# automl/TransformersCanDoBayesianInference

Hardware: AMD Instinct MI355X
Metric: synthetic datasets/sec (GP prior, bptt=2000) (higher is better)
Workload: dtype fp16; 1 GPU; priors.fast_gp, bptt=2000, num_features=18, emsize=512, nhead=4, nhid=1024, nlayers=6, 1000 bars (BASELINE.json configs[1]); per_gpu_batch=64, global_batch=64, aggregate_k_gradients=1, aggregate_streams=0, aggregate_stacked=False, seq_len=2000, parallelism=dp1, micro_batch_streams=2, eval_pos=weighted sampler(2000)

## Files before the change

### transformerscandobayesianinference_amd/csrc/attention.hip

```cpp
#include <algorithm>
#include <type_traits>
#include "pfn_device.h"
#include "pfn_kernels.h"

namespace pfn {

template <typename T, int D> struct AttnCfg {
  static constexpr int RB = D * (int)sizeof(T);
  static constexpr int KVB = (sizeof(T) == 2 && D <= 128) ? 64 : 32;
  static constexpr int NKB = KVB / 32;
  static constexpr int NKK = D / 16;
  static constexpr int NDB = D / 32;
  static constexpr int TILE = KVB * RB;
  static constexpr int RS = PadStride<RB>::ROW, CS = PadStride<RB>::COL;
  static constexpr int RIMG = KVB * RS, CIMG = KVB * CS;
  static constexpr int NW = (sizeof(T) == 2 && D <= 128) ? 8 : 4;
  static constexpr int NT = NW * 64;
  static constexpr int QBLK = NW * 32;
};

template <typename T> PFN_DEV Frag<T> load_frag_global(const T* p) {
  Frag<T> f;
  if constexpr (sizeof(T) == 2) {
    f.v = *reinterpret_cast<const X8<T>*>(p);
// ... 26 lines not shown
    const unsigned w = __builtin_bit_cast(u32x4, f.v)[e >> 1];
    return __builtin_bit_cast(float, (e & 1) ? (w & 0xffff0000u) : (w << 16));
  } else return f.v[e];
}
template <typename T> PFN_DEV float dot8(const Frag<T>& a, const Frag<T>& b) {
  float s = 0.f;
#pragma unroll
  for (int e = 0; e < 8; ++e) s += frag_get(a, e) * frag_get(b, e);
  return s;
}
template <typename T> PFN_DEV f32x4 load4(const T* p) {
  f32x4 r;
  if constexpr (sizeof(T) == 2) {
    X4<T> v = *reinterpret_cast<const X4<T>*>(p);
#pragma unroll
    for (int e = 0; e < 4; ++e) r[e] = (float)v[e];
  } else r = *reinterpret_cast<const f32x4*>(p);
  return r;
}
template <typename T> PFN_DEV void store4(T* p, f32x4 x) {
  if constexpr (sizeof(T) == 2) {
    X4<T> v;
#pragma unroll
    for (int e = 0; e < 4; ++e) v[e] = (T)x[e];
    *reinterpret_cast<X4<T>*>(p) = v;
  } else *reinterpret_cast<f32x4*>(p) = x;
}
PFN_DEV float fast_exp2(float x) { return __builtin_amdgcn_exp2f(x); }

struct AttnBlock { int blk, hd, b; };
PFN_DEV AttnBlock attn_block(int nblk, int H) {
  const int nwg = gridDim.x, bid = blockIdx.x;
  const int q = nwg >> 3, r = nwg & 7, xcd = bid & 7;
  const int id = (xcd < r ? xcd * (q + 1) : r * (q + 1) + (xcd - r) * q) + (bid >> 3);
  AttnBlock o;
  o.blk = id % nblk;
  const int bh = id / nblk;
  o.hd = bh % H;
  o.b = bh / H;
  return o;
}

PFN_DEV AttnBlock attn_block_ragged_last(int nblk, int nfull, int H) {
  if (nfull == nblk) return attn_block(nblk, H);
  const int nwg = gridDim.x, bid = blockIdx.x, npairs = nwg / nblk;
  const int q = nwg >> 3, r = nwg & 7, xcd = bid & 7, j = bid >> 3;
  const int n_x = q + (xcd < r ? 1 : 0);
  const int first = xcd < r ? xcd * (q + 1) : r * (q + 1) + (xcd - r) * q;
  const int r_lo = (int)((long)first * npairs / nwg), r_hi = (int)((long)(first + n_x) * npairs / nwg);
  const int f_x = n_x - (r_hi - r_lo);
  const int f_off = first - r_lo;
  AttnBlock o;
  int pair;
  if (j < f_x) { const int id = f_off + j; pair = id / nfull; o.blk = id % nfull; }
  else { pair = r_lo + (j - f_x); o.blk = nfull; }
  o.hd = pair % H;
  o.b = pair / H;
  return o;
}

typedef __attribute__((address_space(3))) void lvoid_t;
constexpr float LOG2E = 1.4426950408889634f;
constexpr float LN2 = 0.6931471805599453f;
constexpr float RESCALE_THR = 6.f;

PFN_DEV int cache_sep(const int* sep_of, int b, int sep) { return sep_of ? min(max(sep_of[b], 0), sep) : sep; }
PFN_DEV int cache_live_splits(const int* sep_of, int b, int sep, int split_keys, int nsplit) {
  return sep_of ? max(1, min(nsplit, (cache_sep(sep_of, b, sep) + split_keys - 1) / split_keys)) : nsplit;
}

template <typename T> PFN_DEV Frag<T> acc_to_frag_m1(const f32x16& acc, int c, const float (&add8)[8]) {
  static_assert(sizeof(T) == 2, "16-bit operands");
  typedef X2<T> x2;
  const x2 a0 = {(T)(acc[8 * c + 0] + add8[0]), (T)(acc[8 * c + 1] + add8[1])}, a1 = {(T)(acc[8 * c + 2] + add8[2]), (T)(acc[8 * c + 3] + add8[3])};
  const x2 b0 = {(T)(acc[8 * c + 4] + add8[4]), (T)(acc[8 * c + 5] + add8[5])}, b1 = {(T)(acc[8 * c + 6] + add8[6]), (T)(acc[8 * c + 7] + add8[7])};
  const auto r0 = __builtin_amdgcn_permlane32_swap(__builtin_bit_cast(unsigned, a0), __builtin_bit_cast(unsigned, b0), false, false);
  const auto r1 = __builtin_amdgcn_permlane32_swap(__builtin_bit_cast(unsigned, a1), __builtin_bit_cast(unsigned, b1), false, false);
  const u32x4 w = {r0[0], r1[0], r0[1], r1[1]};
  Frag<T> f;
  f.v = __builtin_bit_cast(X8<T>, w);
  return f;
}

template <typename T, int D, bool DROP = false, int DV = D, bool FUSEQ = false, bool CACHE = false>
__global__ __launch_bounds__((AttnCfg<T, D>::NT)) void attn_fwd_kernel(AttnArgs a) {
  static_assert(!CACHE || (!DROP && !FUSEQ), "predict against a cache: no dropout, Q from qkv");
  operand_store_mode<T>();
  using C = AttnCfg<T, D>;
  using CV = AttnCfg<T, DV>;
  static_assert(C::KVB == CV::KVB && D % DV == 0, "V slices share the K tile's key count");
  extern __shared__ __attribute__((aligned(16))) char smem_raw[];
  LdsPtr smem = lds_cast(smem_raw);
  auto Kt = [&](int buf) { return smem + buf * C::RIMG; };
  auto Vt = [&](int buf) { return smem + 2 * C::RIMG + buf * CV::CIMG; };
  constexpr int NVB = 4;
  const int vcol0 = DV == D ? 0 : (int)blockIdx.y * DV;

  AttnBlock wg = attn_block((a.S + C::QBLK - 1) / C::QBLK - a.q_begin / C::QBLK, a.H);
  wg.blk += a.q_begin / C::QBLK;
  const int b = wg.b, hd = wg.hd;
  const int wave = threadIdx.x >> 6, lane = threadIdx.x & 63, h = lane >> 5, li = lane & 31;
  const int lag = (C::NW == 8 && (a.pingpong & 1)) ? (wave >> 2) : 0;
  const long rs = 3L * a.E;
  const T* base = reinterpret_cast<const T*>(a.qkv) + (long)b * a.S * rs;
  const T* Qp = base + hd * D;
  const T* Kp = base + a.E + hd * D;
  const T* Vp = base + 2 * a.E + hd * D + vcol0;
  const int qi = wg.blk * C::QBLK + wave * 32 + li;
  const bool qvalid = qi < a.S;
  const int qc = min(qi, a.S - 1);
  const int k_lo = CACHE ? (int)blockIdx.z * a.split_keys : 0;
  const int sep = CACHE ? min(cache_sep(a.sep_of, b, a.sep) - k_lo, a.split_keys) : a.sep_of ? a.sep_of[b] : a.sep;
  if constexpr (CACHE) { if (blockIdx.z > 0 && sep <= 0) return; }
  const long kld = CACHE ? a.kv_ld : rs;
  const T* Ksrc = CACHE ? reinterpret_cast<const T*>(a.kv) + b * a.kv_sb + k_lo * kld + hd * D : Kp;
  const T* Vsrc = CACHE ? Ksrc + a.E + vcol0 : Vp;
  if (a.q_from_sep && (wg.blk + 1) * C::QBLK <= sep / 256 * 256) return;
  const float scale_log2 = rsqrtf((float)D) * LOG2E;
  const unsigned dseed = DROP ? dropout_pair_seed(a.drop_seed, b * a.H + hd) : 0u;
  const unsigned dthr = DROP ? dropout_threshold(a.p_drop) : 0u;

  Frag<T> qf[C::NKK];
  if constexpr (FUSEQ) {
    static_assert(sizeof(T) == 2 && D <= 128 && C::NW == 8, "fused Q projection: the 8-wave 16-bit configurations");
    constexpr int EC = 128, WS = EC * 2 + 16, WIMG = D * WS;
    static_assert(2 * WIMG <= 2 * C::RIMG + 4 * CV::CIMG, "W_q chunk buffers must fit the (idle) K / V tile buffers");
    const T* xrow = reinterpret_cast<const T*>(a.xq) + ((long)b * a.S + qc) * a.E;
    const T* wq_h = reinterpret_cast<const T*>(a.wq) + (long)(hd * D) * a.E;
    f32x16 qa[C::NDB];
#pragma unroll
    for (int db = 0; db < C::NDB; ++db)
#pragma unroll
      for (int r = 0; r < 16; ++r) qa[db][r] = 0.f;
    TileStage<T, D, EC * 2, C::NT> sw;
    const int nch = a.E / EC;
    sw.issue(wq_h, a.E, D, EC);
    sw.template commit_p<WS>(smem);
    __syncthreads();
    for (int ch = 0; ch < nch; ++ch) {
      const lds_char* wimg = smem + (ch & 1) * WIMG;
      if (ch + 1 < nch) sw.issue(wq_h + (ch + 1) * EC, a.E, D, EC);
      Frag<T> xf[EC / 16];
#pragma unroll
      for (int ks = 0; ks < EC / 16; ++ks) xf[ks] = load_frag_global<T>(xrow + ch * EC + ks * 16 + 8 * h);
#pragma unroll
      for (int ks = 0; ks < EC / 16; ++ks) {
        Frag<T> wf[C::NDB];
#pragma unroll
        for (int db = 0; db < C::NDB; ++db) wf[db] = load_frag_row_p<T, WS>(wimg, db * 32 + li, ks * 16);
#pragma unroll
        for (int db = 0; db < C::NDB; ++db) qa[db] = mma32(wf[db], xf[ks], qa[db]);
      }
      if (ch + 1 < nch) sw.template commit_p<WS>(smem + ((ch + 1) & 1) * WIMG);
      __syncthreads();
    }
    const float* bq = a.bq + hd * D;
    T* qout = reinterpret_cast<T*>(const_cast<void*>(a.qkv)) + (long)b * a.S * rs + hd * D + (long)qc * rs;
#pragma unroll
    for (int db = 0; db < C::NDB; ++db)
#pragma unroll
      for (int c = 0; c < 2; ++c) {
        const f32x4 b0 = *reinterpret_cast<const f32x4*>(bq + db * 32 + 16 * c + 4 * h), b1 = *reinterpret_cast<const f32x4*>(bq + db * 32 + 16 * c + 8 + 4 * h);
        const float add8[8] = {b0[0], b0[1], b0[2], b0[3], b1[0], b1[1], b1[2], b1[3]};
        qf[2 * db + c] = acc_to_frag_m1<T>(qa[db], c, add8);
        if (a.q_store && qvalid) *reinterpret_cast<X8<T>*>(qout + (2 * db + c) * 16 + 8 * h) = qf[2 * db + c].v;
      }
  } else {
#pragma unroll
    for (int kk = 0; kk < C::NKK; ++kk) qf[kk] = load_frag_global<T>(Qp + (long)qc * rs + kk * 16 + 8 * h);
  }

  const bool is_test = CACHE || qc >= sep;
  const bool wave_has_test = CACHE ? blockIdx.z == 0 : wg.blk * C::QBLK + wave * 32 + 31 >= sep;
  float m = -1e30f, lsum = 0.f;
  f32x16 o[CV::NDB];
#pragma unroll
  for (int db = 0; db < CV::NDB; ++db)
#pragma unroll
    for (int r = 0; r < 16; ++r) o[db][r] = 0.f;
  if (wave_has_test) {
    float part = 0.f;
#pragma unroll
    for (int kk = 0; kk < C::NKK; ++kk) part += dot8(qf[kk], load_frag_global<T>(Kp + (long)qc * rs + kk * 16 + 8 * h));
    part += __shfl_xor(part, 32, 64);
    m = is_test ? part * scale_log2 : -1e30f;
    lsum = (is_test && h == 0) ? 1.f : 0.f;
#pragma unroll
    for (int db = 0; db < CV::NDB; ++db)
#pragma unroll
      for (int rg = 0; rg < 4; ++rg) {
        f32x4 v = load4<T>(Vp + (long)qc * rs + db * 32 + 8 * rg + 4 * h);
#pragma unroll
        for (int e = 0; e < 4; ++e) o[db][4 * rg + e] = (is_test && (!DROP || dropout_keep(dseed, (unsigned)qc, (unsigned)qc, dthr))) ? v[e] : 0.f;
      }
  }

  const int nfull = sep / C::KVB;
  const int ntiles = (sep + C::KVB - 1) / C::KVB;
  TileStage<T, C::KVB, C::RB, C::NT> sk;
  TileStage<T, C::KVB, CV::RB, C::NT> sv;
  if (ntiles > 0) {
    sk.issue(Ksrc, kld, sep, D);
    sv.issue(Vsrc, kld, sep, DV);
    sk.template commit_p<C::RS>(Kt(0));
    sv.template commit_p<CV::CS>(Vt(0));
    if (ntiles > 1) {
      sk.issue(Ksrc + (long)C::KVB * kld, kld, sep - C::KVB, D);
      sv.issue(Vsrc + (long)C::KVB * kld, kld, sep - C::KVB, DV);
    }
  }
  __syncthreads();

  constexpr int NPF = C::KVB / 16;
  Frag<T> pf[NPF];
  auto pv_prev = [&](int vb) __attribute__((always_inline)) {
    const lds_char* vt = Vt(vb);
#pragma unroll
    for (int c = 0; c < NPF; ++c)
#pragma unroll
      for (int db = 0; db < CV::NDB; ++db)
        o[db] = mma32(load_frag_tr_p<T, CV::CS, 2>(vt, c * 16, db * 32), pf[c], o[db]);
  };
  int vb_prev = 0, vb_cur = 0;
  for (int t = 0; t < ntiles; ++t) {
    const int k0 = t * C::KVB;
    const lds_char* kt = Kt(t & 1);
    Frag<T> kfr[C::NKK][C::NKB];
#pragma unroll
    for (int kk = 0; kk < C::NKK; ++kk)
#pragma unroll
      for (int kb = 0; kb < C::NKB; ++kb) kfr[kk][kb] = load_frag_row_p<T, C::RS>(kt, kb * 32 + li, kk * 16);
    PFN_PIN_LDS_MFMA();
    f32x16 st[C::NKB];
#pragma unroll
    for (int kb = 0; kb < C::NKB; ++kb)
#pragma unroll
      for (int r = 0; r < 16; ++r) st[kb][r] = 0.f;
#pragma unroll
    for (int kk = 0; kk < C::NKK; ++kk)
#pragma unroll
      for (int kb = 0; kb < C::NKB; ++kb) st[kb] = mma32(kfr[kk][kb], qf[kk], st[kb]);
    PFN_PIN_LDS_MFMA();
    const int vb_next = vb_cur == NVB - 1 ? 0 : vb_cur + 1;
    sk.template commit_p<C::RS>(Kt((t + 1) & 1));
    sv.template commit_p<CV::CS>(Vt(vb_next));
    if (t + 2 < ntiles) {
      const long k2 = k0 + 2 * C::KVB;
      sk.issue(Ksrc + k2 * kld, kld, sep - (int)k2, D);
      sv.issue(Vsrc + k2 * kld, kld, sep - (int)k2, DV);
    }
    if (t == nfull) {
#pragma unroll
      for (int kb = 0; kb < C::NKB; ++kb)
#pragma unroll
        for (int r = 0; r < 16; ++r)
          if (k0 + kb * 32 + acc_row(r, lane) >= sep) st[kb][r] = -INFINITY;
    }
    float mx = -INFINITY;
#pragma unroll
    for (int kb = 0; kb < C::NKB; ++kb)
#pragma unroll
      for (int r = 0; r < 16; ++r) mx = fmaxf(mx, st[kb][r]);
    mx = fmaxf(mx, __shfl_xor(mx, 32, 64));
    const float mc = mx * scale_log2;
    if (__builtin_amdgcn_ballot_w64(mc > m + RESCALE_THR) != 0) {
      const float m_new = fmaxf(m, mc);
      const float alpha = fast_exp2(m - m_new);
      m = m_new;
      lsum *= alpha;
#pragma unroll
      for (int db = 0; db < CV::NDB; ++db)
#pragma unroll
        for (int r = 0; r < 16; ++r) o[db][r] *= alpha;
      if (t > 0) {
#pragma unroll
        for (int c = 0; c < NPF; ++c)
#pragma unroll
          for (int e = 0; e < 8; ++e) pf[c].set(e, frag_get(pf[c], e) * alpha);
      }
    }
    if (lag) __syncthreads();
    if (t > 0) {
      float rsum = 0.f;
#pragma unroll
      for (int kb = 0; kb < C::NKB; ++kb)
#pragma unroll
        for (int r = 0; r < 16; ++r) {
          const float p = fast_exp2(__builtin_fmaf(st[kb][r], scale_log2, -m));
          st[kb][r] = p;
          rsum += p;
        }
      lsum += rsum;
      pv_prev(vb_prev);
    } else {
      float rsum = 0.f;
#pragma unroll
      for (int kb = 0; kb < C::NKB; ++kb)
#pragma unroll
        for (int r = 0; r < 16; ++r) {
          const float p = fast_exp2(__builtin_fmaf(st[kb][r], scale_log2, -m));
          st[kb][r] = p;
          rsum += p;
        }
      lsum += rsum;
    }
    if constexpr (DROP) {
#pragma unroll
      for (int kb = 0; kb < C::NKB; ++kb)
#pragma unroll
        for (int r = 0; r < 16; ++r)
          if (!dropout_keep(dseed, (unsigned)qc, (unsigned)(k0 + kb * 32 + acc_row(r, lane)), dthr)) st[kb][r] = 0.f;
    }
#pragma unroll
    for (int c = 0; c < NPF; ++c) pf[c] = acc_to_frag<T>(st[c >> 1], c & 1);
    vb_prev = vb_cur;
    vb_cur = vb_next;
    if (!lag) __syncthreads();
  }
  if (ntiles > 0) pv_prev(vb_prev);

  lsum += __shfl_xor(lsum, 32, 64);
  if constexpr (CACHE) {
    if (gridDim.z > 1) {
      const long prow = ((long)blockIdx.z * a.B + b) * a.S + qc;
      float* out = a.part_o + prow * a.E + hd * D + vcol0;
#pragma unroll
      for (int db = 0; db < CV::NDB; ++db) {
        float v[16];
#pragma unroll
        for (int r = 0; r < 16; ++r) v[r] = o[db][r];
        store_row_block<float>(out + db * 32, v, h, qvalid);
      }
      if (qvalid && h == 0 && vcol0 == 0) *reinterpret_cast<float2*>(a.part_ml + 2 * (prow * a.H + hd)) = make_float2(m, lsum);
      return;
    }
  }
  const float inv = DROP ? 1.f / (lsum * (1.f - a.p_drop)) : 1.f / lsum;
  {
    T* out = reinterpret_cast<T*>(a.ctx) + ((long)b * a.S + qc) * a.E + hd * D + vcol0;
#pragma unroll
    for (int db = 0; db < CV::NDB; ++db) {
      float v[16];
#pragma unroll
      for (int r = 0; r < 16; ++r) v[r] = o[db][r] * inv;
      store_row_block<T>(out + db * 32, v, h, qvalid);
    }
    if ((!CACHE || a.lse) && qvalid && h == 0 && vcol0 == 0) a.lse[((long)b * a.H + hd) * a.S + qi] = (m + __builtin_amdgcn_logf(lsum)) * LN2;
  }
}

template <typename T>
__global__ __launch_bounds__(256) void attn_merge_kernel(AttnArgs a, int nsplit, int D) {
  const long rows = (long)a.B * a.S, c4n = a.E / 4, total = rows * c4n;
  for (long i = (long)blockIdx.x * 256 + threadIdx.x; i < total; i += (long)gridDim.x * 256) {
    const long row = i / c4n;
    const int c = (int)(i - row * c4n) * 4, hd = c / D;
    const int nz = cache_live_splits(a.sep_of, (int)(row / a.S), a.sep, a.split_keys, nsplit);
    float mx = -INFINITY;
    for (int z = 0; z < nz; ++z) mx = fmaxf(mx, a.part_ml[2 * ((z * rows + row) * a.H + hd)]);
    f32x4 acc = {0.f, 0.f, 0.f, 0.f};
    float l = 0.f;
    for (int z = 0; z < nz; ++z) {
      const float2 ml = *reinterpret_cast<const float2*>(a.part_ml + 2 * ((z * rows + row) * a.H + hd));
      const float w = fast_exp2(ml.x - mx);
      l += w * ml.y;
      const f32x4 v = *reinterpret_cast<const f32x4*>(a.part_o + (z * rows + row) * a.E + c);
#pragma unroll
      for (int e = 0; e < 4; ++e) acc[e] += w * v[e];
    }
    const float inv = 1.f / l;
#pragma unroll
    for (int e = 0; e < 4; ++e) acc[e] *= inv;
    store4<T>(reinterpret_cast<T*>(a.ctx) + row * a.E + c, acc);
    if (a.lse && c % D == 0) a.lse[((row / a.S) * a.H + hd) * a.S + row % a.S] = (mx + __builtin_amdgcn_logf(l)) * LN2;
  }
}

template <typename T, int D> struct BwdCacheCfg {
  static constexpr int DQ = (sizeof(T) == 4 && D == 256) ? 128 : D;
  static constexpr int KVB = 32;
  static constexpr int NKK = D / 16, NDQ = DQ / 32, NPF = KVB / 16;
  static constexpr int RB = D * (int)sizeof(T), QB = DQ * (int)sizeof(T);
  static constexpr int RS = PadStride<RB>::ROW, CSQ = PadStride<QB>::COL;
  static constexpr int KROW = KVB * RS, KCOL = KVB * CSQ;
  static constexpr size_t LDS = 2 * KROW + KCOL;
  static constexpr bool PREFETCH = !(sizeof(T) == 4 && D == 256);
};

template <typename T, int D>
__global__ __launch_bounds__((AttnCfg<T, D>::NT)) void attn_bwd_cache_kernel(AttnCacheBwdArgs a) {
  operand_store_mode<T>();
  using C = AttnCfg<T, D>;
  using G = BwdCacheCfg<T, D>;
  extern __shared__ __attribute__((aligned(16))) char smem_raw[];
  LdsPtr smem = lds_cast(smem_raw);
  LdsPtr Krow = smem, Vrow = smem + G::KROW, Kcol = smem + 2 * G::KROW;
  const AttnBlock wg = attn_block((a.S + C::QBLK - 1) / C::QBLK, a.H);
  const int b = wg.b, hd = wg.hd;
  const int wave = threadIdx.x >> 6, lane = threadIdx.x & 63, h = lane >> 5, li = lane & 31;
  const int qcol0 = G::DQ == D ? 0 : (int)blockIdx.y * G::DQ;
  const long rs = 3L * a.E;
  const int qi = wg.blk * C::QBLK + wave * 32 + li;
// ... 870 lines not shown
  const int sep = a.sep_of ? a.sep_of[b] : a.sep;
  const int qbeg = a.q_from_sep ? sep / 256 * 256 : a.q_begin;
  if ((qb + 1) * P::TB <= qbeg) return;
  const float scale = rsqrtf((float)D), scale_log2 = scale * LOG2E;
  const bool drop = a.p_drop > 0.f;
  const unsigned dseed = dropout_pair_seed(a.drop_seed, b * a.H + hd), dthr = dropout_threshold(a.p_drop);
  const float dscale = drop ? 1.f / (1.f - a.p_drop) : 1.f;
  plain_load_tile<D>(Qs, Qp, rs, q0, qbeg, a.S);
  plain_load_tile<D>(Os, dOp, a.E, q0, qbeg, a.S);
  if (t < P::TB) { const int q = min(q0 + t, a.S - 1); Ls[t] = lse_g[q] * LOG2E; Dl[t] = delta_g[q]; }
  f32x4 dq[D / 32];
#pragma unroll
  for (int m = 0; m < D / 32; ++m) dq[m] = f32x4{0.f, 0.f, 0.f, 0.f};
  const int q = q0 + r1;
  const bool qlive = q >= qbeg && q < a.S;
  for (int key0 = 0; key0 < sep; key0 += P::TB) {
    __syncthreads();
    plain_load_tile<D>(Ks, Kp, rs, key0, 0, sep);
    plain_load_tile<D>(Vs, Vp, rs, key0, 0, sep);
    __syncthreads();
    {
      float s[4], dp[4];
      plain_dots<D>(Qs + r1 * P::RS, Os + r1 * P::RS, Ks, Vs, c1, s, dp);
#pragma unroll
      for (int j = 0; j < 4; ++j) {
        const bool live = qlive && key0 + c1 + j < sep;
        const float p = live ? fast_exp2(s[j] * scale_log2 - Ls[r1]) : 0.f;
        const float mf = !drop ? 1.f : dropout_keep(dseed, (unsigned)q, (unsigned)(key0 + c1 + j), dthr) ? dscale : 0.f;
        Ds[r1 * P::PS + c1 + j] = p * (mf * dp[j] - Dl[r1]);
      }
    }
    __syncthreads();
    for (int kj = 0; kj < P::TB; ++kj) {
      const float ds = Ds[r1 * P::PS + kj];
#pragma unroll
      for (int m = 0; m < D / 32; ++m) {
        const f32x4 k4 = *reinterpret_cast<const f32x4*>(Ks + kj * P::RS + c1 + 32 * m);
#pragma unroll
        for (int e = 0; e < 4; ++e) dq[m][e] += ds * k4[e];
      }
    }
  }
  __syncthreads();
  const bool test = qlive && q >= sep;
  const int qc = min(max(q, 0), a.S - 1);
  float tq = 0.f, dpv = 0.f;
  f32x4 kself[D / 32], vself[D / 32];
#pragma unroll
  for (int m = 0; m < D / 32; ++m) {
    kself[m] = *reinterpret_cast<const f32x4*>(Kp + (long)qc * rs + c1 + 32 * m);
    vself[m] = *reinterpret_cast<const f32x4*>(Vp + (long)qc * rs + c1 + 32 * m);
    const f32x4 q4 = *reinterpret_cast<const f32x4*>(Qs + r1 * P::RS + c1 + 32 * m), o4 = *reinterpret_cast<const f32x4*>(Os + r1 * P::RS + c1 + 32 * m);
#pragma unroll
    for (int e = 0; e < 4; ++e) { tq += q4[e] * kself[m][e]; dpv += o4[e] * vself[m][e]; }
  }
#pragma unroll
  for (int off = 1; off < 8; off <<= 1) { tq += __shfl_xor(tq, off, 64); dpv += __shfl_xor(dpv, off, 64); }
  const float p_self = test ? fast_exp2(tq * scale_log2 - Ls[r1]) : 0.f;
  const float mself = !drop ? 1.f : dropout_keep(dseed, (unsigned)max(q, 0), (unsigned)max(q, 0), dthr) ? dscale : 0.f;
  const float ds_self = p_self * (mself * dpv - Dl[r1]);
  if (qlive) {
#pragma unroll
    for (int m = 0; m < D / 32; ++m) {
      const f32x4 q4 = *reinterpret_cast<const f32x4*>(Qs + r1 * P::RS + c1 + 32 * m), o4 = *reinterpret_cast<const f32x4*>(Os + r1 * P::RS + c1 + 32 * m);
      f32x4 xq, xk, xv;
#pragma unroll
      for (int e = 0; e < 4; ++e) { xq[e] = (dq[m][e] + ds_self * kself[m][e]) * scale; xk[e] = ds_self * scale * q4[e]; xv[e] = p_self * mself * o4[e]; }
      *reinterpret_cast<f32x4*>(dbase + (long)q * rs + hd * D + c1 + 32 * m) = xq;
      if (test) {
        *reinterpret_cast<f32x4*>(dbase + (long)q * rs + a.E + hd * D + c1 + 32 * m) = xk;
        *reinterpret_cast<f32x4*>(dbase + (long)q * rs + 2 * a.E + hd * D + c1 + 32 * m) = xv;
      }
    }
  }
}

bool attn_fwd_can_fuse_q(int E, int H, int precision) {
  const int D = H > 0 ? E / H : 0;
  return prec_is16(precision) && (D == 32 || D == 64 || D == 128) && E % 128 == 0;
}
template <typename T, int D, bool DROP> static int launch_fwd_k(const AttnArgs& a, hipStream_t s) {
  using C = AttnCfg<T, D>;
  constexpr int DV = (sizeof(T) == 4 && D == 256) ? 128 : D;
  constexpr size_t lds = 2 * C::RIMG + 4 * AttnCfg<T, DV>::CIMG;
  static_assert(lds <= 160 * 1024, "attention forward: tile buffers exceed the CU's LDS");
  if ((a.S + C::QBLK - 1) / C::QBLK <= a.q_begin / C::QBLK) return PFN_OK;
  const dim3 grid(((a.S + C::QBLK - 1) / C::QBLK - a.q_begin / C::QBLK) * a.H * a.B, D / DV);
  if constexpr (sizeof(T) == 2 && D <= 128 && !DROP) {
    if (a.xq) {
      if (!a.wq || !a.bq || a.E % 128) return PFN_ERR_ARGUMENT;
      static LdsAllowance allowance_q;
      allowance_q.ensure(attn_fwd_kernel<T, D, false, DV, true>, lds);
      ProfScope ps(PFN_PROF_ATTN_FWD + (a.q_begin > 0 ? 1 : 0), s);
      hipLaunchKernelGGL((attn_fwd_kernel<T, D, false, DV, true>), grid, dim3(C::NT), lds, s, a);
      return hipGetLastError() == hipSuccess ? PFN_OK : PFN_ERR_LAUNCH;
    }
  }
  if (a.xq) return PFN_ERR_UNSUPPORTED;
  static LdsAllowance allowance;
  allowance.ensure(attn_fwd_kernel<T, D, DROP, DV>, lds);
  ProfScope ps(PFN_PROF_ATTN_FWD + (a.q_begin > 0 ? 1 : 0), s);
  hipLaunchKernelGGL((attn_fwd_kernel<T, D, DROP, DV>), grid, dim3(C::NT), lds, s, a);
  return hipGetLastError() == hipSuccess ? PFN_OK : PFN_ERR_LAUNCH;
}
template <typename T, int D> static int launch_fwd_t(const AttnArgs& a, hipStream_t s) {
  return a.p_drop > 0.f ? launch_fwd_k<T, D, true>(a, s) : launch_fwd_k<T, D, false>(a, s);
}
static int g_attn_cache_split_cap = 0;
void set_attn_cache_split_cap(int splits) { g_attn_cache_split_cap = std::max(splits, 0); }
template <typename T, int D> static int launch_fwd_cache_t(const AttnArgs& a_in, hipStream_t s) {
  using C = AttnCfg<T, D>;
  constexpr int DV = (sizeof(T) == 4 && D == 256) ? 128 : D;
  constexpr size_t lds = 2 * C::RIMG + 4 * AttnCfg<T, DV>::CIMG;
  AttnArgs a = a_in;
  int nsplit = attn_cache_splits(a.B, a.S, a.E, a.H, a.sep, sizeof(T) == 4 ? PFN_PREC_F32 : PFN_PREC_BF16);
  if (g_attn_cache_split_cap > 0) nsplit = std::min(nsplit, g_attn_cache_split_cap);
  const int ntiles = (a.sep + C::KVB - 1) / C::KVB;
  a.split_keys = nsplit > 1 ? (ntiles + nsplit - 1) / nsplit * C::KVB : std::max(a.sep, 1);
  const int nz = nsplit > 1 ? (a.sep + a.split_keys - 1) / a.split_keys : 1;
  if (nz > 1 && (!a.part_o || !a.part_ml)) return PFN_ERR_ARGUMENT;
  static LdsAllowance allowance;
  allowance.ensure(attn_fwd_kernel<T, D, false, DV, false, true>, lds);
  const dim3 grid(((a.S + C::QBLK - 1) / C::QBLK) * a.H * a.B, D / DV, nz);
  hipLaunchKernelGGL((attn_fwd_kernel<T, D, false, DV, false, true>), grid, dim3(C::NT), lds, s, a);
  if (nz > 1) {
    const long work = (long)a.B * a.S * (a.E / 4);
    hipLaunchKernelGGL(attn_merge_kernel<T>, dim3((unsigned)std::min<long>((work + 255) / 256, 4096)), dim3(256), 0, s, a, nz, D);
  }
  return hipGetLastError() == hipSuccess ? PFN_OK : PFN_ERR_LAUNCH;
}
template <typename T, int D, bool DROP> static int launch_bwd_k(const AttnArgs& a, hipStream_t s) {
  using C = AttnCfg<T, D>;
  const int parts = a.parts ? a.parts : ~0;
  if (parts & ATTN_BWD_DELTA) {
    const long pairs = (long)a.B * a.S * a.H;
    int grid = (int)std::min<long>((pairs + 15) / 16, 4096);
    ProfScope ps(PFN_PROF_ATTN_BWD_DELTA + (a.q_begin > 0 ? 1 : 0), s);
    hipLaunchKernelGGL(attn_delta_kernel<T>, dim3(grid), dim3(256), 0, s, a, D);
  }
  constexpr size_t lds_kv = BwdKvCfg<T, D>::LDS, lds_dq = BwdDqCfg<T, D>::LDS;
  static_assert(lds_kv <= 160 * 1024 && lds_dq <= 160 * 1024, "attention backward: tile buffers exceed the CU's LDS");
  static LdsAllowance allow_kv, allow_dq;
  if ((parts & ATTN_BWD_KV) && a.sep > 0) {
    ProfScope ps(PFN_PROF_ATTN_BWD_KV + (a.q_begin > 0 ? 1 : 0), s);
    allow_kv.ensure(attn_bwd_kv_kernel<T, D, DROP>, lds_kv);
    hipLaunchKernelGGL((attn_bwd_kv_kernel<T, D, DROP>), dim3(((a.sep + C::QBLK - 1) / C::QBLK) * a.H * a.B), dim3(C::NT), lds_kv, s, a);
  }
  if (parts & ATTN_BWD_DQ) {
    if (a.q_from_sep) {
      const int rc = launch_zero_row_prefix_ragged(a.dqkv, a.S, a.B, a.sep_of, 3L * a.E * (long)sizeof(T), (long)a.E * (long)sizeof(T), s);
      if (rc != PFN_OK) return rc;
    } else if (a.q_begin > 0) {
      const int rc = launch_zero_row_prefix(a.dqkv, a.S, a.B, a.q_begin, 3L * a.E * (long)sizeof(T), (long)a.E * (long)sizeof(T), s);
      if (rc != PFN_OK) return rc;
    }
    if ((a.S + C::QBLK - 1) / C::QBLK <= a.q_begin / C::QBLK) return hipGetLastError() == hipSuccess ? PFN_OK : PFN_ERR_LAUNCH;
    allow_dq.ensure(attn_bwd_dq_kernel<T, D, DROP>, lds_dq);
    ProfScope ps(PFN_PROF_ATTN_BWD_DQ + (a.q_begin > 0 ? 1 : 0), s);
    hipLaunchKernelGGL((attn_bwd_dq_kernel<T, D, DROP>), dim3(((a.S + C::QBLK - 1) / C::QBLK - a.q_begin / C::QBLK) * a.H * a.B), dim3(C::NT), lds_dq, s, a);
  }
  return hipGetLastError() == hipSuccess ? PFN_OK : PFN_ERR_LAUNCH;
}
template <typename T, int D> static int launch_bwd_t(const AttnArgs& a, hipStream_t s) {
  return a.p_drop > 0.f ? launch_bwd_k<T, D, true>(a, s) : launch_bwd_k<T, D, false>(a, s);
}
template <int D> static int launch_bwd_plain_f32(const AttnArgs& a, hipStream_t s) {
  using P = BwdPlainCfg<D>;
  static_assert(P::LDS <= 160 * 1024, "plain attention backward: tiles exceed the CU's LDS");
  const int parts = a.parts ? a.parts : ~0;
  if (parts & ATTN_BWD_DELTA) {
    const long pairs = (long)a.B * a.S * a.H;
    int grid = (int)std::min<long>((pairs + 15) / 16, 4096);
    hipLaunchKernelGGL(attn_delta_kernel<float>, dim3(grid), dim3(256), 0, s, a, D);
  }
  static LdsAllowance allow_kv, allow_dq;
  if ((parts & ATTN_BWD_KV) && a.sep > 0) {
    allow_kv.ensure(attn_bwd_plain_kv_kernel<D>, P::LDS);
    hipLaunchKernelGGL(attn_bwd_plain_kv_kernel<D>, dim3(((a.sep + P::TB - 1) / P::TB) * a.H * a.B), dim3(256), P::LDS, s, a);
  }
  if (parts & ATTN_BWD_DQ) {
    if (a.q_from_sep) {
      const int rc = launch_zero_row_prefix_ragged(a.dqkv, a.S, a.B, a.sep_of, 3L * a.E * 4L, (long)a.E * 4L, s);
      if (rc != PFN_OK) return rc;
    } else if (a.q_begin > 0) {
      const int rc = launch_zero_row_prefix(a.dqkv, a.S, a.B, a.q_begin, 3L * a.E * 4L, (long)a.E * 4L, s);
      if (rc != PFN_OK) return rc;
    }
    const int nqb = (a.S + P::TB - 1) / P::TB - a.q_begin / P::TB;
    if (nqb > 0) {
      allow_dq.ensure(attn_bwd_plain_dq_kernel<D>, P::LDS);
      hipLaunchKernelGGL(attn_bwd_plain_dq_kernel<D>, dim3(nqb * a.H * a.B), dim3(256), P::LDS, s, a);
    }
  }
  return hipGetLastError() == hipSuccess ? PFN_OK : PFN_ERR_LAUNCH;
}

// ... 122 lines not shown
```

### transformerscandobayesianinference_amd/csrc/pfn_device.h

```cpp
#pragma once
#include <hip/hip_runtime.h>
#include <stdint.h>

namespace pfn {

typedef __bf16 bf16;
typedef __attribute__((ext_vector_type(8))) __bf16 bf16x8;
typedef __attribute__((ext_vector_type(4))) __bf16 bf16x4;
typedef __attribute__((ext_vector_type(2))) __bf16 bf16x2;
typedef _Float16 f16;
typedef __attribute__((ext_vector_type(8))) _Float16 f16x8;
typedef __attribute__((ext_vector_type(4))) _Float16 f16x4;
typedef __attribute__((ext_vector_type(2))) _Float16 f16x2;
typedef __attribute__((ext_vector_type(16))) float f32x16;
typedef __attribute__((ext_vector_type(4))) float f32x4;
typedef __attribute__((ext_vector_type(2))) float f32x2;
typedef __attribute__((ext_vector_type(4))) unsigned int u32x4;
typedef __attribute__((ext_vector_type(2))) unsigned int u32x2;
template <typename T> struct OpVec;
template <> struct OpVec<bf16> { typedef bf16x8 x8; typedef bf16x4 x4; typedef bf16x2 x2; };
template <> struct OpVec<f16> { typedef f16x8 x8; typedef f16x4 x4; typedef f16x2 x2; };
template <> struct OpVec<float> { typedef f32x4 x8; typedef f32x4 x4; typedef f32x2 x2; };
template <typename T> using X8 = typename OpVec<T>::x8;
template <typename T> using X4 = typename OpVec<T>::x4;
// ... 183 lines not shown
      if (valid) *reinterpret_cast<f32x4*>(row_block + 8 * rg + 4 * h) = f32x4{v[4 * rg], v[4 * rg + 1], v[4 * rg + 2], v[4 * rg + 3]};
  }
}

template <typename T> PFN_DEV void store_frag_pair_blocked(T* block, const Frag<T>& f0, const Frag<T>& f1, int j, int h, bool valid) {
  char* base = reinterpret_cast<char*>(block);
  if constexpr (sizeof(T) == 2) {
#pragma unroll
    for (int p = 0; p < 2; ++p) {
      const u32x4 d = __builtin_bit_cast(u32x4, p == 0 ? f0.v : f1.v);
      const auto r0 = __builtin_amdgcn_permlane32_swap(d[0], d[2], false, false);
      const auto r1 = __builtin_amdgcn_permlane32_swap(d[1], d[3], false, false);
      const u32x4 w = {r0[0], r1[0], r0[1], r1[1]};
      if (valid) __builtin_nontemporal_store(w, reinterpret_cast<u32x4*>(base + ((p * 32 + j) * 2 + h) * 16));
    }
  } else {
#pragma unroll
    for (int p = 0; p < 2; ++p) {
      const Frag<T>& f = p == 0 ? f0 : f1;
#pragma unroll
      for (int sub = 0; sub < 2; ++sub)
        if (valid) __builtin_nontemporal_store(f32x4{f.v[4 * sub], f.v[4 * sub + 1], f.v[4 * sub + 2], f.v[4 * sub + 3]},
                                               reinterpret_cast<f32x4*>(base + (((2 * p + sub) * 32 + j) * 2 + h) * 16));
    }
  }
}
template <typename T> PFN_DEV int blocked_chunk_row(int w) { return (w >> 1) & 31; }
template <typename T> PFN_DEV int blocked_chunk_col(int w) {
  if constexpr (sizeof(T) == 2) return 16 * (w >> 6) + 8 * (w & 1);
  else return 8 * (w >> 6) + 4 * (w & 1);
}

typedef __amdgpu_buffer_rsrc_t BufRsrc;
PFN_DEV BufRsrc make_rsrc(const void* base, long bytes) {
  const int n = bytes > 0x7ffffff0L ? 0x7ffffff0 : (bytes < 0 ? 0 : (int)bytes);
  return __builtin_amdgcn_make_buffer_rsrc(const_cast<void*>(base), 0, n, 0x00020000);
}
PFN_DEV u32x4 buf_load16(BufRsrc r, int byte_offset) { return __builtin_amdgcn_raw_buffer_load_b128(r, byte_offset, 0, 0); }
constexpr int BUF_OOB = 0x7ffffff0;

struct DmaRsrc { u32x4 w; };
PFN_DEV DmaRsrc make_dma_rsrc(const void* base, long bytes) {
  const unsigned long long p = (unsigned long long)base;
  const int n = bytes > 0x7ffffff0L ? 0x7ffffff0 : (bytes < 0 ? 0 : (int)bytes);
  DmaRsrc r;
  r.w[0] = __builtin_amdgcn_readfirstlane((unsigned)p);
  r.w[1] = __builtin_amdgcn_readfirstlane((unsigned)(p >> 32) & 0xffffu);
  r.w[2] = __builtin_amdgcn_readfirstlane((unsigned)n);
  r.w[3] = 0x00020000u;
  return r;
}
PFN_DEV void dma_rsrc_advance(DmaRsrc& r, unsigned bytes) {
  const unsigned long long b = (((unsigned long long)r.w[1] << 32) | r.w[0]) + bytes;
  r.w[0] = (unsigned)b;
  r.w[1] = (unsigned)(b >> 32);
  r.w[2] = (unsigned)max((int)r.w[2] - (int)bytes, 0);
}
PFN_DEV void dma16(const DmaRsrc& r, LdsPtr lds_dst_uniform, int byte_offset) {
  unsigned keep;
  const unsigned dst = __builtin_amdgcn_readfirstlane((unsigned)(unsigned long long)lds_dst_uniform);
  const u32x4 w = {(unsigned)__builtin_amdgcn_readfirstlane(r.w[0]), (unsigned)__builtin_amdgcn_readfirstlane(r.w[1]),
                   (unsigned)__builtin_amdgcn_readfirstlane(r.w[2]), (unsigned)__builtin_amdgcn_readfirstlane(r.w[3])};
  asm volatile("s_mov_b32 %0, m0\n\ts_mov_b32 m0, %1\n\ts_nop 0\n\tbuffer_load_dwordx4 %2, %3, 0 offen lds\n\ts_mov_b32 m0, %0"
               : "=&s"(keep) : "s"(dst), "v"(byte_offset), "s"(w) : "memory");
}
PFN_DEV void dma4(const DmaRsrc& r, LdsPtr lds_dst_uniform, int byte_offset) {
  unsigned keep;
  const unsigned dst = __builtin_amdgcn_readfirstlane((unsigned)(unsigned long long)lds_dst_uniform);
  const u32x4 w = {(unsigned)__builtin_amdgcn_readfirstlane(r.w[0]), (unsigned)__builtin_amdgcn_readfirstlane(r.w[1]),
                   (unsigned)__builtin_amdgcn_readfirstlane(r.w[2]), (unsigned)__builtin_amdgcn_readfirstlane(r.w[3])};
  asm volatile("s_mov_b32 %0, m0\n\ts_mov_b32 m0, %1\n\ts_nop 0\n\tbuffer_load_dword %2, %3, 0 offen lds\n\ts_mov_b32 m0, %0"
               : "=&s"(keep) : "s"(dst), "v"(byte_offset), "s"(w) : "memory");
}
PFN_DEV void dma16_global(const void* src, LdsPtr lds_dst_uniform) {
  unsigned keep;
  const unsigned dst = __builtin_amdgcn_readfirstlane((unsigned)(unsigned long long)lds_dst_uniform);
  asm volatile("s_mov_b32 %0, m0\n\ts_mov_b32 m0, %1\n\ts_nop 0\n\tglobal_load_lds_dwordx4 %2, off\n\ts_mov_b32 m0, %0"
               : "=&s"(keep) : "s"(dst), "v"(src) : "memory");
}
template <int N> PFN_DEV void wait_vm_barrier() {
  __builtin_amdgcn_s_waitcnt(0x0070 | (N & 15) | ((N >> 4) << 14));
  asm volatile("s_waitcnt vmcnt(%0) lgkmcnt(0)\n\ts_barrier" :: "n"(N) : "memory");
}
PFN_DEV void dma_wait_all() {
  __builtin_amdgcn_s_waitcnt(0x0F70);
  asm volatile("s_waitcnt vmcnt(0)" ::: "memory");
}

template <typename T, int ROWS, int RB, int NT> struct TileStageBuf {
  static constexpr int NCH = RB / 16;
  static constexpr int TOTAL = ROWS * NCH;
  static constexpr int PER = (TOTAL + NT - 1) / NT;
  u32x4 regs[PER];
  int voff[PER];
  PFN_DEV void init(int ld_bytes) {
#pragma unroll
    for (int i = 0; i < PER; ++i) {
      const int id = threadIdx.x + i * NT;
      voff[i] = (TOTAL % NT == 0 || id < TOTAL) ? (id / NCH) * ld_bytes + (id % NCH) * 16 : BUF_OOB;
    }
  }
  PFN_DEV void issue(BufRsrc r, int tile_byte_offset) {
#pragma unroll
    for (int i = 0; i < PER; ++i) regs[i] = buf_load16(r, voff[i] + tile_byte_offset);
  }
  template <int STRIDE> PFN_DEV void commit_p(LdsPtr tile) const {
#pragma unroll
    for (int i = 0; i < PER; ++i) {
      const int id = threadIdx.x + i * NT;
      if (TOTAL % NT != 0 && id >= TOTAL) break;
      lds_write16(tile + (id / NCH) * STRIDE + (id % NCH) * 16, regs[i]);
    }
  }
};

template <typename T, int ROWS, int RB, int NT> struct TileStage {
  static constexpr int NCH = RB / 16;
  static constexpr int TOTAL = ROWS * NCH;
  static constexpr int PER = (TOTAL + NT - 1) / NT;
  static constexpr int EPC = 16 / sizeof(T);
  u32x4 regs[PER];

  PFN_DEV void issue(const T* src, long ld, int rows_valid, int cols_valid) {
#pragma unroll
    for (int i = 0; i < PER; ++i) {
      const int id = threadIdx.x + i * NT;
      const int row = id / NCH, c = id % NCH;
      u32x4 v = {0u, 0u, 0u, 0u};
      if ((TOTAL % NT == 0 || id < TOTAL) && row < rows_valid && (c + 1) * EPC <= cols_valid)
        v = *reinterpret_cast<const u32x4*>(src + (long)row * ld + c * EPC);
      else if ((TOTAL % NT == 0 || id < TOTAL) && row < rows_valid && c * EPC < cols_valid) {
        T tmp[EPC];
#pragma unroll
        for (int e = 0; e < EPC; ++e) tmp[e] = (c * EPC + e < cols_valid) ? src[(long)row * ld + c * EPC + e] : (T)0.f;
        v = *reinterpret_cast<u32x4*>(tmp);
      }
      regs[i] = v;
    }
  }
  template <int STRIDE> PFN_DEV void commit_p(LdsPtr tile) const {
#pragma unroll
    for (int i = 0; i < PER; ++i) {
      const int id = threadIdx.x + i * NT;
      if (TOTAL % NT != 0 && id >= TOTAL) break;
      lds_write16(tile + (id / NCH) * STRIDE + (id % NCH) * 16, regs[i]);
    }
  }
  template <bool SWZ64> PFN_DEV void commit(LdsPtr tile) const {
#pragma unroll
    for (int i = 0; i < PER; ++i) {
      const int id = threadIdx.x + i * NT;
      if (TOTAL % NT != 0 && id >= TOTAL) break;
      const int row = id / NCH, c = id % NCH;
      const int off = SWZ64 ? lds_off64<RB>(row, c * 16) : lds_off16<RB>(row, c);
      lds_write16(tile + off, regs[i]);
    }
  }
};

PFN_DEV float erf_fast(float x) {
  const float ax = fabsf(x);
  const float t = __builtin_amdgcn_rcpf(__builtin_fmaf(0.3275911f, ax, 1.f));
  float p = __builtin_fmaf(1.061405429f, t, -1.453152027f);
  p = __builtin_fmaf(p, t, 1.421413741f);
  p = __builtin_fmaf(p, t, -0.284496736f);
  p = __builtin_fmaf(p, t, 0.254829592f);
// ... 77 lines not shown
```

Before: 2510 datasets/s.

## Stream attention forward K/V tiles into LDS via buffer DMA with triple-buffered K

For the 8-wave 16-bit forward configurations, K/V tile staging moves from register-staged loads plus LDS commits to direct buffer_load-to-LDS DMA. K gets three buffers so the next-next tile can be prefetched, and tile barriers use counted vmcnt waits. This removes register staging and the commit instructions from the inner loop and lets loads overlap compute more deeply. In exchange it uses more LDS, adds a 32-bit span limit check that returns unsupported for large inputs, and carries subtle wait-count correctness risk.

```diff
diff --git a/transformerscandobayesianinference_amd/csrc/attention.hip b/transformerscandobayesianinference_amd/csrc/attention.hip
--- a/transformerscandobayesianinference_amd/csrc/attention.hip
+++ b/transformerscandobayesianinference_amd/csrc/attention.hip
@@ -132,6 +132,65 @@
   return f;
 }
 
+template <typename T, int D, int DV> struct FwdCfg {
+  using C = AttnCfg<T, D>;
+  using CV = AttnCfg<T, DV>;
+  static constexpr bool DMA = C::NW == 8;
+  static constexpr int NKBUF = DMA ? 3 : 2, NVBUF = 4;
+  static constexpr size_t LDS = NKBUF * C::RIMG + NVBUF * CV::CIMG;
+  static constexpr int NPK = C::RIMG / 1024, NPV = CV::CIMG / 1024, NP = NPK + NPV;
+  static constexpr int NI = (NP + C::NW - 1) / C::NW;
+  static constexpr bool ISSUE_FIRST = D < 128;
+  static bool span_ok(long nkeys, long ld) { return !DMA || (nkeys - 1) * ld * (long)sizeof(T) + C::RB <= 0x7ffffff0L; }
+  static_assert(!DMA || (C::RIMG % 1024 == 0 && CV::CIMG % 1024 == 0), "forward tile images must be whole DMA pieces");
+  static_assert(!DMA || NI >= 2, "every wave must own a piece of every batch (the counted wait is never 0 inside the loop)");
+  static_assert(LDS <= 160 * 1024, "attention forward: tile buffers exceed the CU's LDS");
+};
+
+template <typename T, int D, int DV> struct FwdDma {
+  using F = FwdCfg<T, D, DV>;
+  using C = AttnCfg<T, D>;
+  using CV = AttnCfg<T, DV>;
+  DmaRsrc rk, rv;
+  unsigned step;
+  int wave;
+  int pv[F::NI];
+  PFN_DEV void init(const T* Ksrc, const T* Vsrc, long ld, int nkeys, int lane) {
+    wave = __builtin_amdgcn_readfirstlane(threadIdx.x >> 6);
+    const int ldb = (int)(ld * (long)sizeof(T));
+    rk = make_dma_rsrc(Ksrc, ((long)(nkeys - 1) * ld + D) * (long)sizeof(T));
+    rv = make_dma_rsrc(Vsrc, ((long)(nkeys - 1) * ld + DV) * (long)sizeof(T));
+    step = (unsigned)(C::KVB * ldb);
+#pragma unroll
+    for (int i = 0; i < F::NI; ++i) {
+      const int g = wave + C::NW * i;
+      if (C::NW * i + C::NW - 1 < F::NPK || g < F::NPK) {
+        const int byte = g * 1024 + lane * 16, row = byte / C::RS, cb = byte % C::RS;
+        pv[i] = cb < C::RB ? row * ldb + cb : BUF_OOB;
+      } else {
+        const int byte = (g - F::NPK) * 1024 + lane * 16, row = byte / CV::CS, cb = byte % CV::CS;
+        pv[i] = (g < F::NP && cb < CV::RB) ? row * ldb + cb : BUF_OOB;
+      }
+    }
+  }
+  template <bool WITH_V> PFN_DEV void issue(LdsPtr kbuf, LdsPtr vbuf) {
+#pragma unroll
+    for (int i = 0; i < F::NI; ++i) {
+      const int g = wave + C::NW * i;
+      if (C::NW * i + C::NW - 1 < F::NPK || g < F::NPK) dma16(rk, kbuf + g * 1024, pv[i]);
+      else if (WITH_V && (C::NW * i + C::NW - 1 < F::NP || g < F::NP)) dma16(rv, vbuf + (g - F::NPK) * 1024, pv[i]);
+    }
+    dma_rsrc_advance(rk, step);
+    if (WITH_V) dma_rsrc_advance(rv, step);
+  }
+  PFN_DEV void wait_barrier() const {
+    if (F::NP % C::NW == 0 || wave < F::NP % C::NW) dma_wait<F::NI>();
+    else dma_wait<F::NI - 1>();
+    wait_vm_barrier<63>();
+  }
+};
+struct FwdNoDma {};
+
 template <typename T, int D, bool DROP = false, int DV = D, bool FUSEQ = false, bool CACHE = false>
 __global__ __launch_bounds__((AttnCfg<T, D>::NT)) void attn_fwd_kernel(AttnArgs a) {
   static_assert(!CACHE || (!DROP && !FUSEQ), "predict against a cache: no dropout, Q from qkv");
@@ -141,9 +200,10 @@
   static_assert(C::KVB == CV::KVB && D % DV == 0, "V slices share the K tile's key count");
   extern __shared__ __attribute__((aligned(16))) char smem_raw[];
   LdsPtr smem = lds_cast(smem_raw);
+  using F = FwdCfg<T, D, DV>;
   auto Kt = [&](int buf) { return smem + buf * C::RIMG; };
-  auto Vt = [&](int buf) { return smem + 2 * C::RIMG + buf * CV::CIMG; };
-  constexpr int NVB = 4;
+  auto Vt = [&](int buf) { return smem + F::NKBUF * C::RIMG + buf * CV::CIMG; };
+  constexpr int NVB = F::NVBUF;
   const int vcol0 = DV == D ? 0 : (int)blockIdx.y * DV;
 
   AttnBlock wg = attn_block((a.S + C::QBLK - 1) / C::QBLK - a.q_begin / C::QBLK, a.H);
@@ -170,11 +230,21 @@
   const unsigned dseed = DROP ? dropout_pair_seed(a.drop_seed, b * a.H + hd) : 0u;
   const unsigned dthr = DROP ? dropout_threshold(a.p_drop) : 0u;
 
+  typename std::conditional<F::DMA, FwdDma<T, D, DV>, FwdNoDma>::type dma;
+  auto dma_first = [&]() __attribute__((always_inline)) {
+    if constexpr (F::DMA) {
+      dma.init(Ksrc, Vsrc, kld, sep, lane);
+      dma.template issue<true>(Kt(0), Vt(0));
+      dma.template issue<false>(Kt(1), Vt(0));
+    }
+  };
+  if constexpr (!FUSEQ) dma_first();
+
   Frag<T> qf[C::NKK];
   if constexpr (FUSEQ) {
     static_assert(sizeof(T) == 2 && D <= 128 && C::NW == 8, "fused Q projection: the 8-wave 16-bit configurations");
     constexpr int EC = 128, WS = EC * 2 + 16, WIMG = D * WS;
-    static_assert(2 * WIMG <= 2 * C::RIMG + 4 * CV::CIMG, "W_q chunk buffers must fit the (idle) K / V tile buffers");
+    static_assert(2 * WIMG <= F::LDS, "W_q chunk buffers must fit the (idle) K / V tile buffers");
     const T* xrow = reinterpret_cast<const T*>(a.xq) + ((long)b * a.S + qc) * a.E;
     const T* wq_h = reinterpret_cast<const T*>(a.wq) + (long)(hd * D) * a.E;
     f32x16 qa[C::NDB];
@@ -204,6 +274,7 @@
       if (ch + 1 < nch) sw.template commit_p<WS>(smem + ((ch + 1) & 1) * WIMG);
       __syncthreads();
     }
+    dma_first();
     const float* bq = a.bq + hd * D;
     T* qout = reinterpret_cast<T*>(const_cast<void*>(a.qkv)) + (long)b * a.S * rs + hd * D + (long)qc * rs;
 #pragma unroll
@@ -247,19 +318,27 @@
 
   const int nfull = sep / C::KVB;
   const int ntiles = (sep + C::KVB - 1) / C::KVB;
-  TileStage<T, C::KVB, C::RB, C::NT> sk;
-  TileStage<T, C::KVB, CV::RB, C::NT> sv;
-  if (ntiles > 0) {
-    sk.issue(Ksrc, kld, sep, D);
-    sv.issue(Vsrc, kld, sep, DV);
-    sk.template commit_p<C::RS>(Kt(0));
-    sv.template commit_p<CV::CS>(Vt(0));
-    if (ntiles > 1) {
-      sk.issue(Ksrc + (long)C::KVB * kld, kld, sep - C::KVB, D);
-      sv.issue(Vsrc + (long)C::KVB * kld, kld, sep - C::KVB, DV);
-    }
-  }
-  __syncthreads();
+  typename std::conditional<F::DMA, FwdNoDma, TileStage<T, C::KVB, C::RB, C::NT>>::type sk;
+  typename std::conditional<F::DMA, FwdNoDma, TileStage<T, C::KVB, CV::RB, C::NT>>::type sv;
+  if constexpr (F::DMA) {
+    wait_vm_barrier<0>();
+  } else {
+    if (ntiles > 0) {
+      sk.issue(Ksrc, kld, sep, D);
+      sv.issue(Vsrc, kld, sep, DV);
+      sk.template commit_p<C::RS>(Kt(0));
+      sv.template commit_p<CV::CS>(Vt(0));
+      if (ntiles > 1) {
+        sk.issue(Ksrc + (long)C::KVB * kld, kld, sep - C::KVB, D);
+        sv.issue(Vsrc + (long)C::KVB * kld, kld, sep - C::KVB, DV);
+      }
+    }
+    __syncthreads();
+  }
+  auto tile_barrier = [&]() __attribute__((always_inline)) {
+    if constexpr (F::DMA) dma.wait_barrier();
+    else __syncthreads();
+  };
 
   constexpr int NPF = C::KVB / 16;
   Frag<T> pf[NPF];
@@ -272,9 +351,13 @@
         o[db] = mma32(load_frag_tr_p<T, CV::CS, 2>(vt, c * 16, db * 32), pf[c], o[db]);
   };
   int vb_prev = 0, vb_cur = 0;
+  int kb_cur = 0;
   for (int t = 0; t < ntiles; ++t) {
     const int k0 = t * C::KVB;
-    const lds_char* kt = Kt(t & 1);
+    const int vb_next = vb_cur == NVB - 1 ? 0 : vb_cur + 1;
+    const int kb_next = kb_cur == F::NKBUF - 1 ? 0 : kb_cur + 1;
+    if constexpr (F::DMA && F::ISSUE_FIRST) dma.template issue<true>(Kt(kb_next == F::NKBUF - 1 ? 0 : kb_next + 1), Vt(vb_next));
+    const lds_char* kt = Kt(kb_cur);
     Frag<T> kfr[C::NKK][C::NKB];
 #pragma unroll
     for (int kk = 0; kk < C::NKK; ++kk)
@@ -291,13 +374,16 @@
 #pragma unroll
       for (int kb = 0; kb < C::NKB; ++kb) st[kb] = mma32(kfr[kk][kb], qf[kk], st[kb]);
     PFN_PIN_LDS_MFMA();
-    const int vb_next = vb_cur == NVB - 1 ? 0 : vb_cur + 1;
-    sk.template commit_p<C::RS>(Kt((t + 1) & 1));
-    sv.template commit_p<CV::CS>(Vt(vb_next));
-    if (t + 2 < ntiles) {
-      const long k2 = k0 + 2 * C::KVB;
-      sk.issue(Ksrc + k2 * kld, kld, sep - (int)k2, D);
-      sv.issue(Vsrc + k2 * kld, kld, sep - (int)k2, DV);
+    if constexpr (F::DMA) {
+      if constexpr (!F::ISSUE_FIRST) dma.template issue<true>(Kt(kb_next == F::NKBUF - 1 ? 0 : kb_next + 1), Vt(vb_next));
+    } else {
+      sk.template commit_p<C::RS>(Kt(kb_next));
+      sv.template commit_p<CV::CS>(Vt(vb_next));
+      if (t + 2 < ntiles) {
+        const long k2 = k0 + 2 * C::KVB;
+        sk.issue(Ksrc + k2 * kld, kld, sep - (int)k2, D);
+        sv.issue(Vsrc + k2 * kld, kld, sep - (int)k2, DV);
+      }
     }
     if (t == nfull) {
 #pragma unroll
@@ -329,7 +415,7 @@
           for (int e = 0; e < 8; ++e) pf[c].set(e, frag_get(pf[c], e) * alpha);
       }
     }
-    if (lag) __syncthreads();
+    if (lag) tile_barrier();
     if (t > 0) {
       float rsum = 0.f;
 #pragma unroll
@@ -365,9 +451,11 @@
     for (int c = 0; c < NPF; ++c) pf[c] = acc_to_frag<T>(st[c >> 1], c & 1);
     vb_prev = vb_cur;
     vb_cur = vb_next;
-    if (!lag) __syncthreads();
+    kb_cur = kb_next;
+    if (!lag) tile_barrier();
   }
   if (ntiles > 0) pv_prev(vb_prev);
+  if constexpr (F::DMA) dma_wait_all();
 
   lsum += __shfl_xor(lsum, 32, 64);
   if constexpr (CACHE) {
@@ -1404,8 +1492,8 @@
 template <typename T, int D, bool DROP> static int launch_fwd_k(const AttnArgs& a, hipStream_t s) {
   using C = AttnCfg<T, D>;
   constexpr int DV = (sizeof(T) == 4 && D == 256) ? 128 : D;
-  constexpr size_t lds = 2 * C::RIMG + 4 * AttnCfg<T, DV>::CIMG;
-  static_assert(lds <= 160 * 1024, "attention forward: tile buffers exceed the CU's LDS");
+  constexpr size_t lds = FwdCfg<T, D, DV>::LDS;
+  if (!FwdCfg<T, D, DV>::span_ok(a.S, 3L * a.E)) return PFN_ERR_UNSUPPORTED;
   if ((a.S + C::QBLK - 1) / C::QBLK <= a.q_begin / C::QBLK) return PFN_OK;
   const dim3 grid(((a.S + C::QBLK - 1) / C::QBLK - a.q_begin / C::QBLK) * a.H * a.B, D / DV);
   if constexpr (sizeof(T) == 2 && D <= 128 && !DROP) {
@@ -1433,7 +1521,8 @@
 template <typename T, int D> static int launch_fwd_cache_t(const AttnArgs& a_in, hipStream_t s) {
   using C = AttnCfg<T, D>;
   constexpr int DV = (sizeof(T) == 4 && D == 256) ? 128 : D;
-  constexpr size_t lds = 2 * C::RIMG + 4 * AttnCfg<T, DV>::CIMG;
+  constexpr size_t lds = FwdCfg<T, D, DV>::LDS;
+  if (!FwdCfg<T, D, DV>::span_ok(a_in.sep, a_in.kv_ld)) return PFN_ERR_UNSUPPORTED;
   AttnArgs a = a_in;
   int nsplit = attn_cache_splits(a.B, a.S, a.E, a.H, a.sep, sizeof(T) == 4 ? PFN_PREC_F32 : PFN_PREC_BF16);
   if (g_attn_cache_split_cap > 0) nsplit = std::min(nsplit, g_attn_cache_split_cap);
diff --git a/transformerscandobayesianinference_amd/csrc/pfn_device.h b/transformerscandobayesianinference_amd/csrc/pfn_device.h
--- a/transformerscandobayesianinference_amd/csrc/pfn_device.h
+++ b/transformerscandobayesianinference_amd/csrc/pfn_device.h
@@ -289,6 +289,10 @@
   __builtin_amdgcn_s_waitcnt(0x0070 | (N & 15) | ((N >> 4) << 14));
   asm volatile("s_waitcnt vmcnt(%0) lgkmcnt(0)\n\ts_barrier" :: "n"(N) : "memory");
 }
+template <int N> PFN_DEV void dma_wait() {
+  __builtin_amdgcn_s_waitcnt(0x0F70 | (N & 15) | ((N >> 4) << 14));
+  asm volatile("s_waitcnt vmcnt(%0)" :: "n"(N) : "memory");
+}
 PFN_DEV void dma_wait_all() {
   __builtin_amdgcn_s_waitcnt(0x0F70);
   asm volatile("s_waitcnt vmcnt(0)" ::: "memory");
```

New measurement: 2519 datasets/s (median of 6 runs). No clear change (+0.3%).
